# mackelab/poisson-gpfa

Hardware: AMD Instinct MI355X
Metric: EM iterations/sec (higher is better)
Workload: dtype f64

## Files before the change

### poisson-gpfa_amd/csrc/core.hip

```cpp
#include "ctx.h"
#include "model.h"
#include "dual.h"

using namespace pgpfa;

thread_local std::string g_err;
thread_local unsigned long long g_fail_count = 0;

int fail(const char* fmt, ...) {
  char buf[1024];
  va_list ap;
  va_start(ap, fmt);
  vsnprintf(buf, sizeof(buf), fmt, ap);
  va_end(ap);
  g_err = buf;
  ++g_fail_count;
  return 1;
}

int ensure_hbuf(pgpfa_ctx* c, size_t len) {
  if (len <= c->hbuf_len) return 0;
  if (c->hbuf) hipHostFree(c->hbuf);
  c->hbuf = nullptr;
  HIPC(hipHostMalloc((void**)&c->hbuf, len * sizeof(double)));
// ... 827 lines not shown
  {
    const size_t nqmax = (size_t)p * TAU_MULTI_MAX;
    rc |= dmalloc(c, &c->tK, slab * nqmax); rc |= dmalloc(c, &c->tM, slab * nqmax); rc |= dmalloc(c, &c->tA1, slab * nqmax);
    rc |= dmalloc(c, &c->tA2, slab * nqmax);
    rc |= dmalloc(c, &c->tscal, 16 + 8 * nqmax); rc |= dmalloc(c, &c->tpart, 1024 + 64 * nqmax);
  }
  if (rc) { pgpfa_destroy(c); return 1; }
  e = hipStreamSynchronize(c->st);
  if (e != hipSuccess) { pgpfa_destroy(c); return fail("sync: %s", hipGetErrorString(e)); }
  if (const char* g = std::getenv("PGPFA_RANK_GRAN")) { const int v = std::atoi(g); if (v == 4 || v == 8 || v == 16) c->rank_gran = v; }
  c->info["n_pad"] = c->npad;
  c->info["counts_two_bytes"] = 0.0;
  c->info["trial_lengths_set"] = 0.0;
  c->info["observed_set"] = 0.0;
  c->info["observed_bins_set"] = 0.0;
  c->info["last_cd_unobserved_neurons"] = 0.0;
  c->info["arena_bytes"] = 0.0;
  c->info["last_eps_wt_norm"] = 0.0;
  c->info["last_eps_wt_rms"] = 0.0;
  c->info["last_split_cov"] = 0.0;
  c->info["last_syrk_tile"] = 0.0;
  c->info["last_split_sps"] = 0.0;
  c->info["last_cross_kernel"] = 0.0;
  c->info["last_mix_form"] = 0.0;
  c->info["last_yt_mix_fused"] = 0.0;
  c->info["last_cov_f32"] = 0.0;
  c->info["last_cov_f32_fallbacks"] = 0.0;
  for (const char* k : {"plan_ms_total", "plans", "set_params_calls", "last_retry_ms", "last_dense_retries", "last_param_step", "last_param_step_prev",
                        "last_fallback_no_descent", "last_fallback_line_search", "last_fallback_outer_cap", "arena_grow_ms_total", "last_cold_restarts"}) c->info[k] = 0.0;
  *out = c;
  return 0;
}

int pgpfa_destroy(pgpfa_ctx* c) {
  if (!c) return 0;
  hipSetDevice(c->device);
  if (c->st) hipStreamSynchronize(c->st);
  if (c->comm) ncclCommDestroy(c->comm);
  for (void* p : c->allocs) hipFree(p);
  if (c->vsmgp) hipFree(c->vsmgp);
  if (c->Flr32) hipFree(c->Flr32);
  if (c->lam_keep) hipFree(c->lam_keep);
  if (c->split_buf) hipFree(c->split_buf);
  if (c->Yhi) hipFree(c->Yhi);
  if (c->trial_len) hipFree(c->trial_len);
  if (c->obs) hipFree(c->obs);
  if (c->binw) hipFree(c->binw);
  if (c->nlive) hipFree(c->nlive);
  if (c->trunc_q) hipFree(c->trunc_q);
  arena_release(c);
  if (c->hbuf) hipHostFree(c->hbuf);
  if (c->dl_stage) hipHostFree(c->dl_stage);
  if (c->hibuf) hipHostFree(c->hibuf);
  if (c->ring) hipHostFree(c->ring);
  if (c->h_pcg) hipHostFree(c->h_pcg);
  if (c->h_seq) hipHostFree(c->h_seq);
  for (auto e : c->prof.pool) hipEventDestroy(e);
  if (c->st2) { hipStreamSynchronize(c->st2); hipStreamDestroy(c->st2); }
  if (c->tau_pin) hipHostFree(c->tau_pin);
  if (c->ev_tau_fork) hipEventDestroy(c->ev_tau_fork);
  if (c->ev_tau_done) hipEventDestroy(c->ev_tau_done);
  if (c->ev_fork) hipEventDestroy(c->ev_fork);
  if (c->ev_join) hipEventDestroy(c->ev_join);
  if (c->st) hipStreamDestroy(c->st);
  delete c;
  return 0;
}

int pgpfa_set_option(pgpfa_ctx* c, const char* key, double v) {
  if (!c || !key) return fail("null argument");
  const std::string k(key);
  if (k == "newton_xtol") c->xtol = v;
  else if (k == "newton_max_iter") c->max_iter = (int)v;
  else if (k == "use_mfma") {
    const bool was = c->mfma;
    c->mfma = (v != 0.0);
    if (c->have_params && c->rank_gran != 16 && was != c->mfma)
      CHK(pgpfa_set_params(c, std::vector<double>(c->hC).data(), std::vector<double>(c->hd).data(), std::vector<double>(c->htau).data()));
  }
  else if (k == "cd_mfma") c->cd_mfma = (v != 0.0);
  else if (k == "cd_hess_mfma") c->cd_hess_mfma = (v != 0.0);
  else if (k == "cross_kernel") c->cross_kernel = (v != 0.0);
  else if (k == "cd_debug") c->cd_debug = (int)v;
  else if (k == "pcg_fused") c->pcg_fused = (int)v;
  else if (k == "pcg_w32") c->pcg_w32 = (v != 0.0);
  else if (k == "pcg_form") c->pcg_form = (int)v;
  else if (k == "pcg_vec32") c->pcg_vec32 = (int)v;
  else if (k == "pcg_rx32") c->pcg_rx32 = (int)v;
  else if (k == "pcg_adapt") c->pcg_adapt = (int)v;
  else if (k == "pcg_xcd") c->pcg_xcd = (int)v;
  else if (k == "mt_fill") c->mt_fill = (int)v;
  else if (k == "overlap_factors") c->overlap_factors = (int)v;
  else if (k == "mix_slot") c->mix_slot = (int)v;
  else if (k == "yt_mix") c->yt_mix = (v != 0.0);
  else if (k == "pivchol_pairs") c->pivchol_pairs = (v != 0.0);
  else if (k == "vsm_b4") c->vsm_b4 = (int)v;
  else if (k == "poisson_tiles") c->poisson_tiles = (int)v;
  else if (k == "yt_mix_dbg") c->yt_mix_dbg = (int)v;
  else if (k == "yt_mix_dma") c->yt_mix_dma = (v != 0.0);
  else if (k == "syrk_dbg") c->syrk_dbg = (int)v;
  else if (k == "syrk_tile") c->syrk_tile = (int)v;
  else if (k == "mix_wide") c->mix_wide = (int)v;
  else if (k == "thin_products") {
    const bool was = c->thin_products >= 2;
    c->thin_products = (int)v;
// ... 689 lines not shown
```

### poisson-gpfa_amd/csrc/cov.hip

```cpp
#include "ctx.h"
#include "model.h"
#include "split.h"
#include "ytmix.h"

using namespace pgpfa;

template <typename TIN>
void launch_post_vsm(pgpfa_ctx* c, const TIN* Mt, long long sM, int ncol, int ns, int full_range, const int* roff = nullptr, int ts = 0) {
  const int T = c->T, p = c->p;
  if (ts <= 0) ts = T;
  if (p > 10 && c->vsm_mfma) {
    const int CB = post_vsm_mfma_cb(p, sizeof(TIN) == 4);
    if (p <= 20 && c->vsm_b4) {
      constexpr int VW = 16 / (int)sizeof(TIN);
      const bool vec = c->vsm_b4 >= 2 && T % VW == 0 && ts % VW == 0 && c->ld % VW == 0 && sM % VW == 0 && (((size_t)Mt) & 15) == 0;
      auto go = [&](auto nbk, auto vv) {
        constexpr int NBK = decltype(nbk)::value;
        constexpr bool VEC = decltype(vv)::value;
        const size_t lds4 = (size_t)CB * post_vsm_b4_cs(p, VEC) * sizeof(TIN);
        constexpr int BINS = VEC ? 64 : 32;
        (void)hipFuncSetAttribute(reinterpret_cast<const void*>(&post_vsm_b4_kernel<NBK, TIN, VEC>), hipFuncAttributeMaxDynamicSharedMemorySize, (int)lds4);
        hipLaunchKernelGGL((post_vsm_b4_kernel<NBK, TIN, VEC>), dim3((T + BINS - 1) / BINS, ns), dim3(512), lds4, c->st, Mt, sM, c->ld, ncol, T, p, c->vsm,
                           c->ident, c->trial_of_slot, full_range, CB, roff, (int)GBN, ts);
      };
// ... 107 lines not shown
  SyrkF16Args a{};
  a.D = D; a.sD = sD; a.ldd = ldd; a.ts = Ts; a.part = part;
  a.T = T; a.p = p; a.ract = ract; a.nslots = nb; a.sps = sps; a.ngroups = ngroups;
  a.dbg = c->syrk_dbg;
  const int t256 = (T + 255) / 256;
  const bool big = tile_req >= 256 && T > 256 && (Ts & 3) == 0 && (ldd & 3) == 0 && t256 * 256 <= Ts && (((size_t)D) & 15) == 0 && (sD & 3) == 0;
  a.tiles = big ? t256 : (T + 127) / 128; a.ntiles = a.tiles * (a.tiles + 1) / 2;
  const long long blocks = (long long)a.ntiles * ngroups * p;
  prof_begin(c, TAG_VSM, 3.0 * (double)nb * ract * T * T * p);
  if (big) {
    const size_t lds = (size_t)4 * 2 * 256 * 32 * sizeof(_Float16);
    (void)hipFuncSetAttribute(reinterpret_cast<const void*>(&syrk256_f16x2_kernel), hipFuncAttributeMaxDynamicSharedMemorySize, (int)lds);
    hipLaunchKernelGGL(syrk256_f16x2_kernel, dim3((unsigned)blocks), dim3(512), lds, c->st, a);
  } else {
    hipLaunchKernelGGL(syrk_f16x2_kernel, dim3((unsigned)blocks), dim3(256), 0, c->st, a);
  }
  prof_end(c);
  *tile_used = big ? 256 : 128;
  *sps_out = sps;
  *ngroups_out = ngroups;
  return 0;
}

static int split_latent_sums(pgpfa_ctx* c, const double* A0, long long sM, int lda, const float* Dk, long long sD, int ldd, int rk, int kw, int T, int nb, int sps,
                             bool cross, double* Spart, double* Xpart, double* Ssum, double* Xsum, int* cross_used) {
  const int ngroups = (nb + sps - 1) / sps;
  const int spsS = std::max(1, (nb + SPLIT_NS - 1) / SPLIT_NS);
  auto seg = [&](int sper, bool is_x, double* out) -> int {
    const int nfull = nb / sper, rem = nb - nfull * sper;
    for (int part = 0; part < 2; ++part) {
      const int first = part ? nfull * sper : 0, per = part ? rem : sper, ng = part ? (rem ? 1 : 0) : nfull;
      if (ng == 0 || per == 0) continue;
      GemmP g{};
      g.A = A0 + (size_t)first * sM; g.sA = (long long)per * sM; g.lda = lda;
      g.kseg = kw; g.sAseg = sM;
      g.K = per * kw; g.alpha = 1.0; g.beta = 0.0; g.slots = nullptr; g.nbatch = ng; g.kflags = 0; g.bm = 64;
      g.M = rk;
      if (is_x) {
        g.B = reinterpret_cast<const double*>(Dk + (size_t)first * sD);
        g.sB = (long long)per * sD; g.ldb = ldd; g.sBseg = sD; g.b_f32 = 1;
        g.N = T; g.mode = GEMM_FULL;
        g.C = out + (size_t)(part ? nfull : 0) * rk * T; g.sC = (long long)rk * T; g.ldc = rk;
      } else {
        g.B = g.A; g.sB = g.sA; g.ldb = lda; g.sBseg = sM;
        g.N = rk; g.mode = GEMM_LOWER;
        g.C = out + (size_t)(part ? nfull : 0) * rk * rk; g.sC = (long long)rk * rk; g.ldc = rk;
      }
      CHK(gemm(c, false, g));
    }
    return 0;
  };
  CHK(seg(spsS, false, Spart));
  const bool use_cross = cross && c->mfma && rk % 16 == 0 && kw % 16 == 0;
  if (use_cross) {
    for (int row0 = 0; row0 < rk; row0 += 128) {
      CrossArgs ca{};
      ca.A = A0; ca.sM = sM; ca.lda = lda;
      ca.D = Dk; ca.sD = sD; ca.ldd = ldd;
      ca.C = Xpart; ca.sC = (long long)rk * T;
      ca.rk = std::min(128, rk - row0); ca.T = T; ca.kw = kw; ca.nslots = nb; ca.sps = sps;
      ca.row0 = row0; ca.ldc = rk;
      prof_begin(c, TAG_GEMM, 2.0 * (double)nb * ca.rk * (double)kw * T);
      cross_term_launch<float, false>(ca, dim3((T + 63) / 64, ngroups), c->st);
      prof_end(c);
    }
    HIPC(hipGetLastError());
  } else {
    CHK(seg(sps, true, Xpart));
  }
  const int ngS = (nb + spsS - 1) / spsS;
  hipLaunchKernelGGL(sum_groups_kernel, dim3((unsigned)(((size_t)rk * rk + 63) / 64)), dim3(256), 0, c->st, Spart, ngS, rk, rk, 32, Ssum);
  hipLaunchKernelGGL(sum_groups_kernel, dim3((unsigned)(((size_t)rk * T + 63) / 64)), dim3(256), 0, c->st, Xpart, ngroups, rk, T, 0, Xsum);
  *cross_used = use_cross ? 1 : 0;
  return 0;
}

static int accumulate_split(pgpfa_ctx* c, const CholWS& lw, int nb, int ract, int Ts, bool skip_zero_cols, int ctile, bool fused) {
  const int T = c->T, p = c->p, Tp = c->Tp, rpad = c->rpad;
  const long long sW = (long long)T * p * p;
  const size_t tt = (size_t)T * T;
  (void)skip_zero_cols;
  constexpr int NS = SPLIT_NS, NG = PACC_SPLITS + 1;
  const size_t tq = (size_t)round_up(T, 16) * round_up(T, 16);
  if (!c->split_buf) {
    const size_t len = ((size_t)NS + NG + 3) * tq + 2 * (size_t)p * tt + 1024;
    if (hipMalloc((void**)&c->split_buf, len * sizeof(double)) != hipSuccess) { (void)hipGetLastError(); c->split_buf = nullptr; return fail("out of device memory for the split accumulation (%zu bytes)", len * sizeof(double)); }
    c->bytes += len * sizeof(double);
  }
  double* Spart = c->split_buf;
  double* Xpart = Spart + (size_t)NS * tq;
  double* Ssum = Xpart + (size_t)NG * tq;
  double* Xsum = Ssum + tq;
  double* Zb = Xsum + tq;
  double* T1 = Zb + tq;
  double* Xfull = T1 + (size_t)p * tt;
// ... 51 lines not shown
                           c->Gbin, sW, T, ract, c->eps, c->vsm, c->ident, c->trial_of_slot, c->d_roff, ctile, Ts);
        mix_form = 2;
        return;
      }
      if (c->mix_slot) {
        (void)hipFuncSetAttribute(reinterpret_cast<const void*>(&mix_slot_kernel<PW, 256, 2>), hipFuncAttributeMaxDynamicSharedMemorySize, (int)mix_slot_lds(PW, 256));
        hipLaunchKernelGGL((mix_slot_kernel<PW, 256, 2>), dim3((T + 255) / 256, nb), dim3(256), mix_slot_lds(PW, 256), c->st, (const double*)lw.H, (long long)lw.sH, c->ld, D, sD, ldd,
                           c->Gbin, sW, T, p, ract, c->eps, c->vsm, c->ident, c->trial_of_slot, c->d_roff, ctile, Ts);
        mix_form = 1;
        return;
      }
    }
    if constexpr (PW <= 16)
      hipLaunchKernelGGL(mix_vsm_split_kernel<PW>, dim3((T + 63) / 64, nb), dim3(256), 0, c->st, (const double*)lw.H, (long long)lw.sH, c->ld, D, sD, ldd,
                         c->Gbin, sW, T, p, ract, c->eps, c->vsm, c->ident, c->trial_of_slot, c->d_roff, ctile, Ts);
  });
  prof_end(c);
  }
  c->info["last_mix_form"] = (double)mix_form;
  int sps = 0, ngroups = 0, tile_used = 0;
  CHK(split_syrk_launch(c, D, sD, ldd, Ts, T, p, ract, nb, 0, c->syrk_tile, c->ppart, &tile_used, &sps, &ngroups));
  c->info["last_syrk_tile"] = (double)tile_used;
  c->info["last_split_sps"] = (double)sps;
  bool cross_ran = false;
  for (int k = 0; k < p; ++k) {
    const int rk = c->rk[k], r0 = c->roff[k] & ~15;
    const int rrow = c->roff[k];
    const int kw = ract - r0;
    if (kw <= 0 || rk <= 0) {
      HIPC(hipMemsetAsync(T1 + (size_t)k * tt, 0, tt * sizeof(double), c->st));
      HIPC(hipMemsetAsync(Xfull + (size_t)k * tt, 0, tt * sizeof(double), c->st));
      continue;
    }
    const double* A0 = lw.Mt + rrow + (size_t)r0 * rpad;
    int cross_used = 0;
    CHK(split_latent_sums(c, A0, (long long)lw.sM, rpad, D + (size_t)k * Ts + (size_t)r0 * ldd, sD, ldd, rk, kw, T, nb, sps, c->cross_kernel, Spart, Xpart, Ssum, Xsum,
                          &cross_used));
    cross_ran = cross_ran || cross_used != 0;
    const double* Fk = c->Flr + (size_t)k * Tp * Tp;
    GemmP z{};
    z.A = Fk; z.lda = Tp; z.B = Ssum; z.ldb = rk; z.C = Zb; z.ldc = T;
    z.M = T; z.N = rk; z.K = rk; z.alpha = 1.0; z.beta = 0.0; z.nbatch = 1; z.mode = GEMM_FULL;
    CHK(gemm(c, true, z));
    GemmP t1 = z;
    t1.A = Zb; t1.lda = T; t1.B = Fk; t1.ldb = Tp; t1.C = T1 + (size_t)k * tt; t1.ldc = T; t1.N = T;
    CHK(gemm(c, false, t1));
    GemmP xf = z;
    xf.B = Xsum; xf.ldb = rk; xf.C = Xfull + (size_t)k * tt; xf.ldc = T; xf.N = T;
    CHK(gemm(c, true, xf));
  }
  c->info["last_cross_kernel"] = cross_ran ? 1.0 : 0.0;
  {
    const int nt64 = (T + PACC_TS - 1) / PACC_TS;
    hipLaunchKernelGGL(pacc_split_reduce_kernel, dim3(nt64 * (nt64 + 1) / 2, p), dim3(256), 0, c->st, T1, Xfull, c->ppart, ngroups, c->Gbin, sW, nb, c->eps, T, Tp,
                       p, c->Pacc);
  }
  HIPC(hipGetLastError());
  c->pacc_used = true;
  return 0;
}

static int posterior_blocks_lowrank_impl(pgpfa_ctx* c, int nb, bool want_vsmgp, bool accumulate, double* logdet_out, bool allow_lap32, double* ld_dev) {
  const int T = c->T, p = c->p, Tp = c->Tp, pp = p * p;
  const int rpad = c->rpad;
  const int ract = round_up(c->rtot, 16);
  const long long sW = (long long)T * pp;
  c->last_cov_lowrank = true;
  CHK(bin_blocks(c, c->W, sW, c->Gbin, c->Wt, sW, nb, (logdet_out || ld_dev) ? c->ldet_buf : nullptr));
  const bool split_candidate = want_vsmgp && accumulate && c->split_cov && c->mfma && (p <= 16 || (p <= 20 && c->mix_wide));
  unsigned* norm_bits = reinterpret_cast<unsigned*>(c->pcg_ratio);
  if (split_candidate || c->measure_mix) {
    HIPC(hipMemsetAsync(norm_bits, 0, 4 * sizeof(unsigned), c->st));
    const long long nblk = (long long)nb * T;
    hipLaunchKernelGGL(block_norm_max_kernel, dim3((unsigned)std::min<long long>((nblk * p + 255) / 256, 2048)), dim3(256), 0, c->st, c->Wt, nblk, p, c->eps, norm_bits,
// ... 149 lines not shown
    c->info["last_eps_wt_rms"] = std::max(c->info["last_eps_wt_rms"], rms);
    split = split_candidate && std::isfinite(hv) && std::isfinite(rms) && rms <= c->split_max_norm && (double)hv <= 0.9;
    return 0;
  };
  const bool fuse_candidate = split_candidate && c->yt_mix && c->mfma && p <= 10 && (ract == c->rtot || (c->rank_compact && ract <= lw.nact));
  if (fuse_candidate) CHK(decide_split());
  const bool fused = fuse_candidate && split;
  c->info["last_yt_mix_fused"] = fused ? 1.0 : 0.0;
  if (!fused) {
    for (int k = 0; k < p; ++k) {
      const int c0 = skip_zero_cols ? (c->roff[k] / ctile) * ctile : 0;
      if (c0 >= ract) continue;
      GemmP g{};
      g.A = c->Flr + (size_t)k * Tp * Tp; g.sA = 0; g.lda = Tp;
      g.B = lw.Mt + c->roff[k] + (size_t)c0 * rpad; g.sB = lw.sM; g.ldb = rpad;
      g.C = lw.H + (size_t)k * Ts + (size_t)c0 * c->ld; g.sC = lw.sH; g.ldc = c->ld;
      g.M = T; g.N = ract - c0; g.K = c->rk[k]; g.alpha = 1.0; g.beta = 0.0;
      g.slots = c->ident; g.nbatch = nb; g.mode = GEMM_FULL; g.kflags = 0;
      CHK(gemm(c, true, g));
    }
  }
  if (!decided) CHK(decide_split());
  c->info["last_split_cov"] = split ? 1.0 : 0.0;
  if (!split) for (const char* key : {"last_syrk_tile", "last_split_sps", "last_cross_kernel", "last_mix_form"}) c->info[key] = 0.0;
  if (want_vsmgp && split) {
    CHK(accumulate_split(c, lw, nb, ract, Ts, skip_zero_cols, ctile, fused));
  } else if (want_vsmgp) {
    prof_begin(c, TAG_MIX, (double)nb * c->n * ract * 16.0);
    dispatch_pw(p, [&](auto pw) {
      constexpr int PW = decltype(pw)::value;
      if constexpr (PW <= 16) {
        hipLaunchKernelGGL(mix_vsm_kernel<PW>, dim3((T + 63) / 64, nb), dim3(256), 0, c->st, lw.H, lw.sH, c->ld, c->Gbin, sW, T, p, ract, c->eps,
                           c->vsm, c->ident, c->trial_of_slot, c->d_roff, ctile, Ts);
      } else if (c->mix_wide && p <= 20) {
        hipLaunchKernelGGL((mix_vsm_wide2_kernel<20, false>), dim3((T + 63) / 64, nb), dim3(256), 0, c->st, lw.H, (long long)lw.sH, c->ld, c->Gbin, sW, T, p, ract, c->eps,
                           c->vsm, c->ident, c->trial_of_slot, Ts, c->sink, (float*)nullptr, 0LL, 0);
      } else {
        const int bins = wide_bins(p);
        hipLaunchKernelGGL(mix_vsm_wide_kernel, dim3((T + bins - 1) / bins, nb), dim3(bins * 32), wide_lds_bytes(p, bins, 1), c->st, lw.H, lw.sH,
                           c->ld, c->Gbin, sW, T, p, ract, c->eps, c->vsm, c->ident, c->trial_of_slot, bins, Ts);
      }
    });
    prof_end(c);
  } else {
    prof_begin(c, TAG_VSM, (double)nb * c->n * rpad * p);
    launch_post_vsm(c, (const double*)lw.H, (long long)lw.sH, ract, nb, 1, skip_zero_cols ? c->d_roff : nullptr, Ts);
    prof_end(c);
// ... 294 lines not shown
  float* dD = nullptr;
  double* dpart = nullptr;
  CHK(hb.get(&dD, slot * nslots, 1024));
  HIPC(hipMemcpy(dD, D, slot * nslots * sizeof(float), hipMemcpyHostToDevice));
  CHK(hook_output(hb, &dpart, part, np));
  int sps_used = 0;
  CHK(split_syrk_launch(c, dD, (long long)slot, ldd, ts, T, p, ract, nslots, sps, tile, dpart, tile_used, &sps_used, ngroups));
  HIPC(hipGetLastError());
  HIPC(hipStreamSynchronize(c->st));
  return hook_collect("pgpfa_test_split_syrk", dpart, part, np);
}

int pgpfa_test_split_latent_sums(pgpfa_ctx* c, int nslots, int rk, int kw, int T, int lda, long long sM, int row_off, int ldd, long long sD, int sps, int cross_kernel,
                                 const double* A, const float* D, double* Ssum, double* Xsum) {
  if (!c || !A || !D || !Ssum || !Xsum) return fail("null argument");
  if (nslots < 1 || T < 1 || rk < 1 || kw < 1 || sps < 0 || row_off < 0) return fail("invalid sizes");
  if (rk % 16 != 0) return fail("rk = %d is no multiple of 16", rk);
  if (kw % 16 != 0) return fail("kw = %d is no multiple of 16", kw);
  if (lda < row_off + rk) return fail("lda = %d below row_off + rk = %d", lda, row_off + rk);
  if (ldd < T) return fail("ldd = %d below T = %d", ldd, T);
  if (sM < (long long)kw * lda || sD < (long long)kw * ldd) return fail("slot strides below kw columns");
  if (!c->mfma) return fail("the split form runs on the matrix cores (use_mfma = 1)");
  const int sps_eff = sps > 0 ? sps : std::max(1, (nslots + PACC_SPLITS - 1) / PACC_SPLITS);
  const int ng = (nslots + sps_eff - 1) / sps_eff;
  const int spsS = std::max(1, (nslots + SPLIT_NS - 1) / SPLIT_NS), ngS = (nslots + spsS - 1) / spsS;
  HIPC(hipSetDevice(c->device));
  HIPC(hipStreamSynchronize(c->st));
  HookBuffers hb;
  double *dA = nullptr, *dSp = nullptr, *dXp = nullptr, *dS = nullptr, *dX = nullptr;
  float* dD = nullptr;
  CHK(hb.get(&dA, (size_t)sM * nslots, 4096));
  CHK(hb.get(&dD, (size_t)sD * nslots, 4096));
  CHK(hb.get(&dSp, (size_t)ngS * rk * rk, 1024));
  CHK(hb.get(&dXp, (size_t)ng * rk * T, 1024));
  HIPC(hipMemcpy(dA, A, (size_t)sM * nslots * sizeof(double), hipMemcpyHostToDevice));
  HIPC(hipMemcpy(dD, D, (size_t)sD * nslots * sizeof(float), hipMemcpyHostToDevice));
  CHK(hook_output(hb, &dS, Ssum, (size_t)rk * rk));
  CHK(hook_output(hb, &dX, Xsum, (size_t)rk * T));
  int cross_used = 0;
  CHK(split_latent_sums(c, dA + row_off, sM, lda, dD, sD, ldd, rk, kw, T, nslots, sps_eff, cross_kernel != 0, dSp, dXp, dS, dX, &cross_used));
  HIPC(hipGetLastError());
  HIPC(hipStreamSynchronize(c->st));
  if ((cross_kernel != 0) != (cross_used != 0)) return fail("internal: the cross term did not take the requested form");
  CHK(hook_collect("pgpfa_test_split_latent_sums (S)", dS, Ssum, (size_t)rk * rk));
  return hook_collect("pgpfa_test_split_latent_sums (X)", dX, Xsum, (size_t)rk * T);
}
```

### poisson-gpfa_amd/csrc/ctx.h

```cpp
#pragma once
#include <hip/hip_runtime.h>
#include <rccl/rccl.h>

#include <algorithm>
#include <limits>
#include <chrono>
#include <cmath>
#include <cstdarg>
#include <cstdio>
#include <cstring>
#include <deque>
#include <functional>
#include <map>
#include <string>
#include <type_traits>
#include <vector>

#include <mutex>
#include <rocprofiler-sdk-roctx/roctx.h>
#include "../../include/pgpfa.h"
#include "types.h"

using namespace pgpfa;

// ... 186 lines not shown
  bool plan_lowrank = false;
  size_t slab_elems = 0, mt_elems = 0, ws_mark = 0;
  char* arena = nullptr; size_t arena_cap = 0, arena_off = 0; int arena_mode = 0;
  int vmm = 0; size_t va_size = 0, vmm_gran = 0, vmm_granule = (size_t)1 << 30;
  std::vector<std::pair<hipMemGenericAllocationHandle_t, size_t>> vmm_chunks;
  double arena_headroom = 2.0;
  bool mt_dirty = false;
  bool last_cov_lowrank = false;
  bool shared_pcg = true;
  bool pcg_trace = false;
  double* zero16 = nullptr;
  double* sink = nullptr;
  int mix_wide = 1;
  int poisson_tiles = 2;
  int vsm_b4 = 2;
  int pivchol_pairs = 1;
  int yt_mix = 1;
  int syrk_tile = 256;
  int syrk_dbg = 0;
  int yt_mix_dma = 1;
  int yt_mix_dbg = 0;
  int mix_slot = 3;
  bool cross_kernel = true;
  bool measure_mix = false;
  bool time_newton = false;
  int shared_min = 16, pcg_inner_min = 2, pcg_inner_max = 16, pcg_outer_max = 12;
  double pcg_eta0 = 1e-2;
  int splitk_target = 1280;
  int f32_tile64 = 1;
  int small_tile_below = 1 << 30;
  int splitk_below64 = 400;
  double *sc_f = nullptr, *sc_qxx = nullptr, *sc_qdx = nullptr, *sc_qdd = nullptr, *sc_dec = nullptr, *sc_smax = nullptr, *sc_alpha = nullptr;
  int *trial_of_slot = nullptr, *list_a = nullptr, *list_b = nullptr, *ident = nullptr;
  int* mask_of_slot = nullptr;
  bool mask_active = false;
  CholWS kws{};
  double *tK = nullptr, *tM = nullptr, *tA1 = nullptr, *tA2 = nullptr, *tscal = nullptr, *tpart = nullptr;
  double* hbuf = nullptr; size_t hbuf_len = 0;
  struct DlEntry { void* host; size_t off, bytes; };
  PcgCtl fused_ctl_host{};
  char* dl_stage = nullptr; size_t dl_used = 0; std::vector<DlEntry> dl_pending;
  char* dl_stage_dev = nullptr; char* ring_dev = nullptr;
  unsigned* h_seq = nullptr; unsigned* d_seq = nullptr; unsigned seq_next = 0;
  bool copy_kernels = true;
  unsigned long long dl_fail_mark = 0;
  int* hibuf = nullptr; size_t hibuf_len = 0;
// ... 167 lines not shown
```

### poisson-gpfa_amd/csrc/split.h

```cpp
#pragma once
#include <type_traits>
#include <hip/hip_runtime.h>

namespace pgpfa {

typedef _Float16 half8_t __attribute__((ext_vector_type(8)));
typedef float float4v_t __attribute__((ext_vector_type(4)));

constexpr float SPLIT_SCALE = 2048.0f;


template <int PW>
__global__ __launch_bounds__(256, 2) void mix_vsm_split_kernel(const double* __restrict__ Yt, long long sY, int ldy, float* __restrict__ D, long long sD,
                                                            int ldd, const double* __restrict__ G, long long sG, int T, int p, int rpad, double eps,
                                                            double* __restrict__ vsm, const int* __restrict__ slots,
                                                            const int* __restrict__ trial_of_slot, const int* __restrict__ roff, int col_tile, int ts) {
  constexpr int PP = PW * PW, LD = PP + 1, NPAIR = PW * (PW + 1) / 2;
  __shared__ double Gs[64 * LD];
  const int pp = p * p;
  const int slot = slots[blockIdx.y];
  const int t0 = blockIdx.x * 64;
  const int nt = min(64, T - t0);
  const double* gbase = G + (size_t)slot * sG + (size_t)t0 * pp;
  if (p < PW)
// ... 652 lines not shown
  if (!wave_live) return;
  double* C = a.part + (size_t)(k * a.ngroups + g) * a.T * a.T;
  const double inv = 1.0 / ((double)SPLIT_SCALE * (double)SPLIT_SCALE);
#pragma unroll
  for (int mi = 0; mi < 4; ++mi) {
    const int i = i0 + wm * 64 + mi * 16 + l15;
    if (i >= a.T) continue;
#pragma unroll
    for (int ni = 0; ni < 8; ++ni)
#pragma unroll
      for (int r = 0; r < 4; ++r) {
        const int j = j0 + wn * 128 + ni * 16 + 4 * l4 + r;
        if (j >= a.T) continue;
        C[(size_t)j * a.T + i] = (double)acc[mi][ni][r] * inv;
      }
  }
}

struct CrossArgs {
  const double* A; long long sM; int lda;
  const void* D; long long sD; int ldd;
  double* C; long long sC;
  int rk, T, kw, nslots, sps;
  int row0, ldc;
};

template <int NTR, typename TB, bool LOWER>
__global__ __launch_bounds__(256) void cross_term_kernel(CrossArgs a) {
  constexpr int GK = 16;
  constexpr int RS = NTR * 16 + ((NTR & 1) ? 0 : 16);
  constexpr int NA = (GK * NTR * 16 + 255) / 256;
  __shared__ double As[2][GK][RS];
  __shared__ double Bs[2][GK][64 + 16];
  const int tid = threadIdx.x;
  const int lane = tid & 63, wave = __builtin_amdgcn_readfirstlane(tid >> 6);
  const int l15 = lane & 15, l4 = lane >> 4;
  const int t0 = blockIdx.x * 64;
  const int g = blockIdx.y;
  const int s_begin = g * a.sps, s_end = min(a.nslots, s_begin + a.sps);
  const int cps = a.kw / GK;
  const int nchunks = (s_end - s_begin) * cps;
  const int rk = a.rk;
  const TB* Dall = reinterpret_cast<const TB*>(a.D);
  const int ct = blockIdx.x * 4 + wave;
  const bool wave_live = t0 + wave * 16 < a.T;

  double raA[NA], raB[NA];
  TB rbA[4], rbB[4];
  int cur_s = s_begin, cur_c = 0;
  size_t aoff[NA], doff[4];
#pragma unroll
  for (int u = 0; u < NA; ++u) {
    const int e = tid + 256 * u;
    const int kk = min(e / (NTR * 16), GK - 1), i = min(e % (NTR * 16), rk - 1);
    aoff[u] = (size_t)kk * a.lda + i;
  }
#pragma unroll
  for (int u = 0; u < 4; ++u) {
    const int e = tid + 256 * u;
    const int kk = e >> 6, t = min(t0 + (e & 63), a.T - 1) - t0;
    doff[u] = (size_t)kk * a.ldd + t;
  }
  auto load = [&](int, double (&ra)[NA], TB (&rb)[4]) {
    const int c0 = cur_c * GK;
    const double* Ap = a.A + (size_t)cur_s * a.sM + (size_t)c0 * a.lda + a.row0;
    const TB* Dp = Dall + (size_t)cur_s * a.sD + (size_t)c0 * a.ldd + t0;
#pragma unroll
    for (int u = 0; u < NA; ++u) ra[u] = Ap[aoff[u]];
#pragma unroll
    for (int u = 0; u < 4; ++u) rb[u] = Dp[doff[u]];
    if (cur_c + 1 < cps) ++cur_c;
    else if (cur_s + 1 < s_end) { ++cur_s; cur_c = 0; }
  };
  auto store = [&](int buf, const double (&ra)[NA], const TB (&rb)[4]) {
#pragma unroll
    for (int u = 0; u < NA; ++u) {
      const int e = tid + 256 * u;
      const int kk = e / (NTR * 16), i = e - kk * (NTR * 16);
      if (kk < GK) As[buf][kk][i] = (i < rk) ? ra[u] : 0.0;
    }
#pragma unroll
    for (int u = 0; u < 4; ++u) {
      const int e = tid + 256 * u;
      Bs[buf][e >> 6][e & 63] = (t0 + (e & 63) < a.T) ? (double)rb[u] : 0.0;
    }
  };
  mdouble4 acc[NTR];
#pragma unroll
  for (int mi = 0; mi < NTR; ++mi) acc[mi] = mdouble4{0.0, 0.0, 0.0, 0.0};
  auto multiply = [&](int buf) {
    if (!wave_live) return;
#pragma unroll
    for (int kk = 0; kk < GK; kk += 4) {
      const double bf = Bs[buf][kk + l4][wave * 16 + l15];
#pragma unroll
      for (int mi = 0; mi < NTR; ++mi)
        if (!LOWER || mi >= ct) acc[mi] = __builtin_amdgcn_mfma_f64_16x16x4f64(bf, As[buf][kk + l4][mi * 16 + l15], acc[mi], 0, 0, 0);
    }
  };
  if (nchunks > 0) {
    load(0, raA, rbA);
    load(1, raB, rbB);
    store(0, raA, rbA);
  }
  __syncthreads();
  for (int ch = 0; ch < nchunks; ch += 2) {
    load(ch + 2, raA, rbA);
    multiply(0);
    if (ch + 1 < nchunks) store(1, raB, rbB);
    __syncthreads();
    if (ch + 1 >= nchunks) break;
    load(ch + 3, raB, rbB);
    multiply(1);
    if (ch + 2 < nchunks) store(0, raA, rbA);
    __syncthreads();
  }
  if (!wave_live) return;
  double* C = a.C + (size_t)g * a.sC + a.row0;
#pragma unroll
  for (int mi = 0; mi < NTR; ++mi) {
    const int i = mi * 16 + l15;
    if (i >= rk || (LOWER && mi < ct)) continue;
#pragma unroll
    for (int r = 0; r < 4; ++r) {
      const int t = t0 + wave * 16 + l4 + 4 * r;
      if (t < a.T) C[(size_t)t * a.ldc + i] = acc[mi][r];
    }
  }
}

template <typename TB, bool LOWER>
inline void cross_term_launch(const CrossArgs& ca, dim3 grid, hipStream_t st) {
  switch (ca.rk / 16) {
    case 1: hipLaunchKernelGGL((cross_term_kernel<1, TB, LOWER>), grid, dim3(256), 0, st, ca); break;
    case 2: hipLaunchKernelGGL((cross_term_kernel<2, TB, LOWER>), grid, dim3(256), 0, st, ca); break;
    case 3: hipLaunchKernelGGL((cross_term_kernel<3, TB, LOWER>), grid, dim3(256), 0, st, ca); break;
    case 4: hipLaunchKernelGGL((cross_term_kernel<4, TB, LOWER>), grid, dim3(256), 0, st, ca); break;
    case 5: hipLaunchKernelGGL((cross_term_kernel<5, TB, LOWER>), grid, dim3(256), 0, st, ca); break;
    case 6: hipLaunchKernelGGL((cross_term_kernel<6, TB, LOWER>), grid, dim3(256), 0, st, ca); break;
    case 7: hipLaunchKernelGGL((cross_term_kernel<7, TB, LOWER>), grid, dim3(256), 0, st, ca); break;
    default: hipLaunchKernelGGL((cross_term_kernel<8, TB, LOWER>), grid, dim3(256), 0, st, ca); break;
  }
}

inline __global__ __launch_bounds__(256) void sum_groups_kernel(const double* __restrict__ part, int ngroups, int M, int N, int lower, double* __restrict__ out) {
  __shared__ double red[4][64];
  const int el = threadIdx.x & 63, q = threadIdx.x >> 6;
  const size_t e = (size_t)blockIdx.x * 64 + el;
  const bool in = e < (size_t)M * N;
  const size_t ec = in ? e : 0;
  const int i = (int)(ec % M), j = (int)(ec / M);
  const size_t src = (lower > 0 && (i / lower) < (j / lower)) ? (size_t)i * M + j : ec;
  const size_t gs = (size_t)M * N;
  double s8[8] = {0.0, 0.0, 0.0, 0.0, 0.0, 0.0, 0.0, 0.0};
  int g = q;
  for (; g + 28 < ngroups; g += 32) {
    double v[8];
#pragma unroll
    for (int u = 0; u < 8; ++u) v[u] = part[(size_t)(g + 4 * u) * gs + src];
#pragma unroll
    for (int u = 0; u < 8; ++u) s8[u] += v[u];
  }
  for (; g < ngroups; g += 4) s8[0] += part[(size_t)g * gs + src];
  red[q][el] = ((s8[0] + s8[1]) + (s8[2] + s8[3])) + ((s8[4] + s8[5]) + (s8[6] + s8[7]));
  __syncthreads();
  if (q == 0 && in) out[e] = (red[0][el] + red[1][el]) + (red[2][el] + red[3][el]);
}

constexpr int PACC_TS = 32;
inline __global__ __launch_bounds__(256) void pacc_split_reduce_kernel(const double* __restrict__ T1, const double* __restrict__ X, const double* __restrict__ DD, int ngroups,
                                                                const double* __restrict__ G, long long sG, int nslots, double eps, int T, int Tp, int p,
                                                                double* __restrict__ Pacc) {
  constexpr int TS = PACC_TS;
  __shared__ double Xa[TS][TS + 1], Xb[TS][TS + 1], Ss[TS][TS + 1];
  __shared__ double gd[TS];
  const int k = blockIdx.y;
  int tj = 0, rem = blockIdx.x;
  const int ntile = (T + TS - 1) / TS;
  while (rem >= ntile - tj) { rem -= ntile - tj; ++tj; }
  const int ti = tj + rem;
  const int i0 = ti * TS, j0 = tj * TS;
  const size_t tt = (size_t)T * T;
  const double* t1 = T1 + (size_t)k * tt;
  const double* x = X + (size_t)k * tt;
  const double* dd = DD + (size_t)k * ngroups * tt;
  double* out = Pacc + (size_t)k * Tp * Tp;
  const int tid = threadIdx.x;
  for (int e = tid; e < TS * TS; e += 256) {
    const int r = e % TS, cc = e / TS;
// ... 40 lines not shown
```

Baseline: 12.49.

## Size cross-term groups to occupancy, widen column tiles, batch split tail GEMMs

```diff
diff --git a/poisson-gpfa_amd/csrc/core.hip b/poisson-gpfa_amd/csrc/core.hip
--- a/poisson-gpfa_amd/csrc/core.hip
+++ b/poisson-gpfa_amd/csrc/core.hip
@@ -873,6 +873,7 @@
   c->info["last_syrk_tile"] = 0.0;
   c->info["last_split_sps"] = 0.0;
   c->info["last_cross_kernel"] = 0.0;
+  c->info["last_cross_groups"] = 0.0;
   c->info["last_mix_form"] = 0.0;
   c->info["last_yt_mix_fused"] = 0.0;
   c->info["last_cov_f32"] = 0.0;
@@ -893,6 +894,7 @@
   if (c->Flr32) hipFree(c->Flr32);
   if (c->lam_keep) hipFree(c->lam_keep);
   if (c->split_buf) hipFree(c->split_buf);
+  if (c->split_tail) hipFree(c->split_tail);
   if (c->Yhi) hipFree(c->Yhi);
   if (c->trial_len) hipFree(c->trial_len);
   if (c->obs) hipFree(c->obs);
@@ -932,6 +934,10 @@
   else if (k == "cd_mfma") c->cd_mfma = (v != 0.0);
   else if (k == "cd_hess_mfma") c->cd_hess_mfma = (v != 0.0);
   else if (k == "cross_kernel") c->cross_kernel = (v != 0.0);
+  else if (k == "cross_groups") c->cross_groups = std::max(0, (int)v);
+  else if (k == "cross_xcd") c->cross_xcd = (v != 0.0) ? 1 : 0;
+  else if (k == "cross_bins") c->cross_bins = (v >= 128.0) ? 128 : 64;
+  else if (k == "split_tail_batched") c->split_tail_batched = (v != 0.0) ? 1 : 0;
   else if (k == "cd_debug") c->cd_debug = (int)v;
   else if (k == "pcg_fused") c->pcg_fused = (int)v;
   else if (k == "pcg_w32") c->pcg_w32 = (v != 0.0);
diff --git a/poisson-gpfa_amd/csrc/cov.hip b/poisson-gpfa_amd/csrc/cov.hip
--- a/poisson-gpfa_amd/csrc/cov.hip
+++ b/poisson-gpfa_amd/csrc/cov.hip
@@ -153,9 +153,32 @@
   return 0;
 }
 
+static bool split_use_cross(const pgpfa_ctx* c, bool cross, int rk, int kw) { return cross && c->mfma && rk % 16 == 0 && kw % 16 == 0; }
+
+static int split_x_groups(pgpfa_ctx* c, bool use_cross, int rk, int T, int nb, int sps, long long cap, int* spsx) {
+  if (!use_cross) { *spsx = sps; return (nb + sps - 1) / sps; }
+  int want = c->cross_groups;
+  if (want <= 0) {
+    if (c->num_cu <= 0) {
+      int n = 0;
+      if (hipDeviceGetAttribute(&n, hipDeviceAttributeMultiprocessorCount, c->device) != hipSuccess) { (void)hipGetLastError(); n = 0; }
+      c->num_cu = n > 0 ? n : 256;
+    }
+    const int rk0 = std::min(rk, 128), nct = cross_term_nct(rk0, T, c->cross_bins);
+    const int occ = std::max(1, cross_term_occupancy<float, false>(rk0 / 16, nct));
+    const int nbt = (T + 64 * nct - 1) / (64 * nct);
+    want = round_up((c->num_cu * occ + nbt - 1) / nbt, 8);
+  }
+  want = (int)std::max<long long>(1, std::min<long long>(std::min<long long>(want, nb), cap));
+  *spsx = (nb + want - 1) / want;
+  return (nb + *spsx - 1) / *spsx;
+}
+
 static int split_latent_sums(pgpfa_ctx* c, const double* A0, long long sM, int lda, const float* Dk, long long sD, int ldd, int rk, int kw, int T, int nb, int sps,
-                             bool cross, double* Spart, double* Xpart, double* Ssum, double* Xsum, int* cross_used) {
-  const int ngroups = (nb + sps - 1) / sps;
+                             bool cross, long long xcap, double* Spart, double* Xpart, double* Ssum, double* Xsum, int ldo, bool merge_sums, int* cross_used) {
+  const bool use_cross = split_use_cross(c, cross, rk, kw);
+  int spsx = sps;
+  const int ngroups = split_x_groups(c, use_cross, rk, T, nb, sps, xcap, &spsx);
   const int spsS = std::max(1, (nb + SPLIT_NS - 1) / SPLIT_NS);
   auto seg = [&](int sper, bool is_x, double* out) -> int {
     const int nfull = nb / sper, rem = nb - nfull * sper;
@@ -182,26 +205,34 @@
     return 0;
   };
   CHK(seg(spsS, false, Spart));
-  const bool use_cross = cross && c->mfma && rk % 16 == 0 && kw % 16 == 0;
   if (use_cross) {
     for (int row0 = 0; row0 < rk; row0 += 128) {
       CrossArgs ca{};
       ca.A = A0; ca.sM = sM; ca.lda = lda;
       ca.D = Dk; ca.sD = sD; ca.ldd = ldd;
       ca.C = Xpart; ca.sC = (long long)rk * T;
-      ca.rk = std::min(128, rk - row0); ca.T = T; ca.kw = kw; ca.nslots = nb; ca.sps = sps;
+      ca.rk = std::min(128, rk - row0); ca.T = T; ca.kw = kw; ca.nslots = nb; ca.sps = spsx;
+      ca.nct = cross_term_nct(ca.rk, T, c->cross_bins);
+      ca.ngroups = ngroups; ca.nbt = (T + 64 * ca.nct - 1) / (64 * ca.nct); ca.xcd = c->cross_xcd;
       ca.row0 = row0; ca.ldc = rk;
       prof_begin(c, TAG_GEMM, 2.0 * (double)nb * ca.rk * (double)kw * T);
-      cross_term_launch<float, false>(ca, dim3((T + 63) / 64, ngroups), c->st);
+      cross_term_launch<float, false>(ca, c->st);
       prof_end(c);
     }
     HIPC(hipGetLastError());
+    c->info["last_cross_groups"] = (double)ngroups;
   } else {
     CHK(seg(sps, true, Xpart));
   }
   const int ngS = (nb + spsS - 1) / spsS;
-  hipLaunchKernelGGL(sum_groups_kernel, dim3((unsigned)(((size_t)rk * rk + 63) / 64)), dim3(256), 0, c->st, Spart, ngS, rk, rk, 32, Ssum);
-  hipLaunchKernelGGL(sum_groups_kernel, dim3((unsigned)(((size_t)rk * T + 63) / 64)), dim3(256), 0, c->st, Xpart, ngroups, rk, T, 0, Xsum);
+  const SumGroupsJob js{Spart, ngS, rk, rk, 32, Ssum, ldo}, jx{Xpart, ngroups, rk, T, 0, Xsum, ldo};
+  const unsigned nblkS = (unsigned)(((size_t)rk * rk + 63) / 64), nblkX = (unsigned)(((size_t)rk * T + 63) / 64);
+  if (merge_sums) {
+    hipLaunchKernelGGL(sum_groups_kernel, dim3(nblkS + nblkX), dim3(256), 0, c->st, js, jx, (int)nblkS);
+  } else {
+    hipLaunchKernelGGL(sum_groups_kernel, dim3(nblkS), dim3(256), 0, c->st, js, js, (int)nblkS);
+    hipLaunchKernelGGL(sum_groups_kernel, dim3(nblkX), dim3(256), 0, c->st, jx, jx, (int)nblkX);
+  }
   *cross_used = use_cross ? 1 : 0;
   return 0;
 }
@@ -299,21 +330,43 @@
   CHK(split_syrk_launch(c, D, sD, ldd, Ts, T, p, ract, nb, 0, c->syrk_tile, c->ppart, &tile_used, &sps, &ngroups));
   c->info["last_syrk_tile"] = (double)tile_used;
   c->info["last_split_sps"] = (double)sps;
+  int rmax = 0;
+  for (int k = 0; k < p; ++k) rmax = std::max(rmax, c->rk[k]);
+  const bool batched = c->split_tail_batched && rmax > 0 && rmax <= Tp;
+  const size_t sS = (size_t)rmax * rmax, sX = (size_t)rmax * T;
+  if (batched) {
+    const size_t ra = (size_t)std::min(round_up(rmax, 64), std::max(rmax, round_up(T, 16)));
+    const size_t need = (size_t)p * (ra * ra + 2 * ra * T) + 1024;
+    if (need > c->split_tail_len) {
+      if (c->split_tail) { HIPC(hipStreamSynchronize(c->st)); HIPC(hipFree(c->split_tail)); c->bytes -= c->split_tail_len * sizeof(double); c->split_tail = nullptr; c->split_tail_len = 0; }
+      if (hipMalloc((void**)&c->split_tail, need * sizeof(double)) != hipSuccess) { (void)hipGetLastError(); c->split_tail = nullptr; return fail("out of device memory for the batched tail of the split accumulation (%zu bytes)", need * sizeof(double)); }
+      c->split_tail_len = need;
+      c->bytes += need * sizeof(double);
+    }
+    HIPC(hipMemsetAsync(c->split_tail, 0, (size_t)p * (sS + sX) * sizeof(double), c->st));
+  }
+  double* SsumB = c->split_tail;
+  double* XsumB = batched ? SsumB + (size_t)p * sS : nullptr;
+  double* ZB = batched ? XsumB + (size_t)p * sX : nullptr;
+  const long long xcap = (long long)NG * (long long)tq;
   bool cross_ran = false;
   for (int k = 0; k < p; ++k) {
     const int rk = c->rk[k], r0 = c->roff[k] & ~15;
     const int rrow = c->roff[k];
     const int kw = ract - r0;
     if (kw <= 0 || rk <= 0) {
+      if (batched) continue;
       HIPC(hipMemsetAsync(T1 + (size_t)k * tt, 0, tt * sizeof(double), c->st));
       HIPC(hipMemsetAsync(Xfull + (size_t)k * tt, 0, tt * sizeof(double), c->st));
       continue;
     }
     const double* A0 = lw.Mt + rrow + (size_t)r0 * rpad;
     int cross_used = 0;
-    CHK(split_latent_sums(c, A0, (long long)lw.sM, rpad, D + (size_t)k * Ts + (size_t)r0 * ldd, sD, ldd, rk, kw, T, nb, sps, c->cross_kernel, Spart, Xpart, Ssum, Xsum,
-                          &cross_used));
+    CHK(split_latent_sums(c, A0, (long long)lw.sM, rpad, D + (size_t)k * Ts + (size_t)r0 * ldd, sD, ldd, rk, kw, T, nb, sps, c->cross_kernel,
+                          xcap / ((long long)rk * T), Spart, Xpart, batched ? SsumB + (size_t)k * sS : Ssum, batched ? XsumB + (size_t)k * sX : Xsum,
+                          batched ? rmax : rk, batched, &cross_used));
     cross_ran = cross_ran || cross_used != 0;
+    if (batched) continue;
     const double* Fk = c->Flr + (size_t)k * Tp * Tp;
     GemmP z{};
     z.A = Fk; z.lda = Tp; z.B = Ssum; z.ldb = rk; z.C = Zb; z.ldc = T;
@@ -326,7 +379,20 @@
     xf.B = Xsum; xf.ldb = rk; xf.C = Xfull + (size_t)k * tt; xf.ldc = T; xf.N = T;
     CHK(gemm(c, true, xf));
   }
+  if (batched) {
+    GemmP z{};
+    z.A = c->Flr; z.sA = (long long)Tp * Tp; z.lda = Tp; z.B = SsumB; z.sB = (long long)sS; z.ldb = rmax; z.C = ZB; z.sC = (long long)sX; z.ldc = T;
+    z.M = T; z.N = rmax; z.K = rmax; z.alpha = 1.0; z.beta = 0.0; z.slots = nullptr; z.nbatch = p; z.mode = GEMM_FULL;
+    CHK(gemm(c, true, z));
+    GemmP t1 = z;
+    t1.A = ZB; t1.sA = (long long)sX; t1.lda = T; t1.B = c->Flr; t1.sB = (long long)Tp * Tp; t1.ldb = Tp; t1.C = T1; t1.sC = (long long)tt; t1.ldc = T; t1.N = T;
+    CHK(gemm(c, false, t1));
+    GemmP xf = z;
+    xf.B = XsumB; xf.sB = (long long)sX; xf.ldb = rmax; xf.C = Xfull; xf.sC = (long long)tt; xf.ldc = T; xf.N = T;
+    CHK(gemm(c, true, xf));
+  }
   c->info["last_cross_kernel"] = cross_ran ? 1.0 : 0.0;
+  if (!cross_ran) c->info["last_cross_groups"] = 0.0;
   {
     const int nt64 = (T + PACC_TS - 1) / PACC_TS;
     hipLaunchKernelGGL(pacc_split_reduce_kernel, dim3(nt64 * (nt64 + 1) / 2, p), dim3(256), 0, c->st, T1, Xfull, c->ppart, ngroups, c->Gbin, sW, nb, c->eps, T, Tp,
@@ -522,7 +588,7 @@
   }
   if (!decided) CHK(decide_split());
   c->info["last_split_cov"] = split ? 1.0 : 0.0;
-  if (!split) for (const char* key : {"last_syrk_tile", "last_split_sps", "last_cross_kernel", "last_mix_form"}) c->info[key] = 0.0;
+  if (!split) for (const char* key : {"last_syrk_tile", "last_split_sps", "last_cross_kernel", "last_cross_groups", "last_mix_form"}) c->info[key] = 0.0;
   if (want_vsmgp && split) {
     CHK(accumulate_split(c, lw, nb, ract, Ts, skip_zero_cols, ctile, fused));
   } else if (want_vsmgp) {
@@ -863,9 +929,11 @@
   if (sM < (long long)kw * lda || sD < (long long)kw * ldd) return fail("slot strides below kw columns");
   if (!c->mfma) return fail("the split form runs on the matrix cores (use_mfma = 1)");
   const int sps_eff = sps > 0 ? sps : std::max(1, (nslots + PACC_SPLITS - 1) / PACC_SPLITS);
-  const int ng = (nslots + sps_eff - 1) / sps_eff;
   const int spsS = std::max(1, (nslots + SPLIT_NS - 1) / SPLIT_NS), ngS = (nslots + spsS - 1) / spsS;
   HIPC(hipSetDevice(c->device));
+  const long long xcap = std::max(1, nslots);
+  int spsx = 0;
+  const int ng = split_x_groups(c, split_use_cross(c, cross_kernel != 0, rk, kw), rk, T, nslots, sps_eff, xcap, &spsx);
   HIPC(hipStreamSynchronize(c->st));
   HookBuffers hb;
   double *dA = nullptr, *dSp = nullptr, *dXp = nullptr, *dS = nullptr, *dX = nullptr;
@@ -879,7 +947,7 @@
   CHK(hook_output(hb, &dS, Ssum, (size_t)rk * rk));
   CHK(hook_output(hb, &dX, Xsum, (size_t)rk * T));
   int cross_used = 0;
-  CHK(split_latent_sums(c, dA + row_off, sM, lda, dD, sD, ldd, rk, kw, T, nslots, sps_eff, cross_kernel != 0, dSp, dXp, dS, dX, &cross_used));
+  CHK(split_latent_sums(c, dA + row_off, sM, lda, dD, sD, ldd, rk, kw, T, nslots, sps_eff, cross_kernel != 0, xcap, dSp, dXp, dS, dX, rk, false, &cross_used));
   HIPC(hipGetLastError());
   HIPC(hipStreamSynchronize(c->st));
   if ((cross_kernel != 0) != (cross_used != 0)) return fail("internal: the cross term did not take the requested form");
diff --git a/poisson-gpfa_amd/csrc/ctx.h b/poisson-gpfa_amd/csrc/ctx.h
--- a/poisson-gpfa_amd/csrc/ctx.h
+++ b/poisson-gpfa_amd/csrc/ctx.h
@@ -232,6 +232,13 @@
   int yt_mix_dbg = 0;
   int mix_slot = 3;
   bool cross_kernel = true;
+  int cross_groups = 0;
+  int cross_xcd = 1;
+  int cross_bins = 128;
+  int split_tail_batched = 1;
+  int num_cu = 0;
+  double* split_tail = nullptr;
+  size_t split_tail_len = 0;
   bool measure_mix = false;
   bool time_newton = false;
   int shared_min = 16, pcg_inner_min = 2, pcg_inner_max = 16, pcg_outer_max = 12;
diff --git a/poisson-gpfa_amd/csrc/split.h b/poisson-gpfa_amd/csrc/split.h
--- a/poisson-gpfa_amd/csrc/split.h
+++ b/poisson-gpfa_amd/csrc/split.h
@@ -698,33 +698,48 @@
   const void* D; long long sD; int ldd;
   double* C; long long sC;
   int rk, T, kw, nslots, sps;
+  int ngroups, nbt, xcd;
+  int nct;
   int row0, ldc;
 };
 
-template <int NTR, typename TB, bool LOWER>
+template <int NTR, typename TB, bool LOWER, int NCT = 1>
 __global__ __launch_bounds__(256) void cross_term_kernel(CrossArgs a) {
+  static_assert(NCT == 1 || (NCT == 2 && !LOWER), "two column tiles per wave: the cross term only");
   constexpr int GK = 16;
   constexpr int RS = NTR * 16 + ((NTR & 1) ? 0 : 16);
   constexpr int NA = (GK * NTR * 16 + 255) / 256;
+  constexpr int BW = 64 * NCT;
+  constexpr int NBV = GK * BW / 256;
+  typedef typename std::conditional<NCT == 2, TB, double>::type TS;
   __shared__ double As[2][GK][RS];
-  __shared__ double Bs[2][GK][64 + 16];
+  __shared__ TS Bs[2][GK][BW + 16];
   const int tid = threadIdx.x;
   const int lane = tid & 63, wave = __builtin_amdgcn_readfirstlane(tid >> 6);
   const int l15 = lane & 15, l4 = lane >> 4;
-  const int t0 = blockIdx.x * 64;
-  const int g = blockIdx.y;
+  int bt, g;
+  {
+    const int id = blockIdx.x;
+    if (a.xcd) { const int m = id >> 3; const int q = m / a.nbt; bt = m - q * a.nbt; g = (id & 7) + 8 * q; }
+    else { g = id / a.nbt; bt = id - g * a.nbt; }
+  }
+  if (g >= a.ngroups) return;
+  const int t0 = bt * BW;
   const int s_begin = g * a.sps, s_end = min(a.nslots, s_begin + a.sps);
   const int cps = a.kw / GK;
   const int nchunks = (s_end - s_begin) * cps;
   const int rk = a.rk;
   const TB* Dall = reinterpret_cast<const TB*>(a.D);
-  const int ct = blockIdx.x * 4 + wave;
-  const bool wave_live = t0 + wave * 16 < a.T;
+  const int ct = bt * 4 + wave;
+  bool live[NCT];
+#pragma unroll
+  for (int c = 0; c < NCT; ++c) live[c] = t0 + c * 64 + wave * 16 < a.T;
+  const bool wave_live = live[0];
 
   double raA[NA], raB[NA];
-  TB rbA[4], rbB[4];
+  TB rbA[NBV], rbB[NBV];
   int cur_s = s_begin, cur_c = 0;
-  size_t aoff[NA], doff[4];
+  size_t aoff[NA], doff[NBV];
 #pragma unroll
   for (int u = 0; u < NA; ++u) {
     const int e = tid + 256 * u;
@@ -732,23 +747,23 @@
     aoff[u] = (size_t)kk * a.lda + i;
   }
 #pragma unroll
-  for (int u = 0; u < 4; ++u) {
+  for (int u = 0; u < NBV; ++u) {
     const int e = tid + 256 * u;
-    const int kk = e >> 6, t = min(t0 + (e & 63), a.T - 1) - t0;
+    const int kk = e / BW, t = min(t0 + (e % BW), a.T - 1) - t0;
     doff[u] = (size_t)kk * a.ldd + t;
   }
-  auto load = [&](int, double (&ra)[NA], TB (&rb)[4]) {
+  auto load = [&](int, double (&ra)[NA], TB (&rb)[NBV]) {
     const int c0 = cur_c * GK;
     const double* Ap = a.A + (size_t)cur_s * a.sM + (size_t)c0 * a.lda + a.row0;
     const TB* Dp = Dall + (size_t)cur_s * a.sD + (size_t)c0 * a.ldd + t0;
 #pragma unroll
     for (int u = 0; u < NA; ++u) ra[u] = Ap[aoff[u]];
 #pragma unroll
-    for (int u = 0; u < 4; ++u) rb[u] = Dp[doff[u]];
+    for (int u = 0; u < NBV; ++u) rb[u] = Dp[doff[u]];
     if (cur_c + 1 < cps) ++cur_c;
     else if (cur_s + 1 < s_end) { ++cur_s; cur_c = 0; }
   };
-  auto store = [&](int buf, const double (&ra)[NA], const TB (&rb)[4]) {
+  auto store = [&](int buf, const double (&ra)[NA], const TB (&rb)[NBV]) {
 #pragma unroll
     for (int u = 0; u < NA; ++u) {
       const int e = tid + 256 * u;
@@ -756,22 +771,31 @@
       if (kk < GK) As[buf][kk][i] = (i < rk) ? ra[u] : 0.0;
     }
 #pragma unroll
-    for (int u = 0; u < 4; ++u) {
+    for (int u = 0; u < NBV; ++u) {
       const int e = tid + 256 * u;
-      Bs[buf][e >> 6][e & 63] = (t0 + (e & 63) < a.T) ? (double)rb[u] : 0.0;
-    }
-  };
-  mdouble4 acc[NTR];
-#pragma unroll
-  for (int mi = 0; mi < NTR; ++mi) acc[mi] = mdouble4{0.0, 0.0, 0.0, 0.0};
+      Bs[buf][e / BW][e % BW] = (t0 + (e % BW) < a.T) ? (TS)rb[u] : (TS)0;
+    }
+  };
+  mdouble4 acc[NCT][NTR];
+#pragma unroll
+  for (int c = 0; c < NCT; ++c)
+#pragma unroll
+    for (int mi = 0; mi < NTR; ++mi) acc[c][mi] = mdouble4{0.0, 0.0, 0.0, 0.0};
   auto multiply = [&](int buf) {
     if (!wave_live) return;
 #pragma unroll
     for (int kk = 0; kk < GK; kk += 4) {
-      const double bf = Bs[buf][kk + l4][wave * 16 + l15];
-#pragma unroll
-      for (int mi = 0; mi < NTR; ++mi)
-        if (!LOWER || mi >= ct) acc[mi] = __builtin_amdgcn_mfma_f64_16x16x4f64(bf, As[buf][kk + l4][mi * 16 + l15], acc[mi], 0, 0, 0);
+      double bf[NCT];
+#pragma unroll
+      for (int c = 0; c < NCT; ++c) bf[c] = (double)Bs[buf][kk + l4][c * 64 + wave * 16 + l15];
+#pragma unroll
+      for (int mi = 0; mi < NTR; ++mi) {
+        if (LOWER && mi < ct) continue;
+        const double af = As[buf][kk + l4][mi * 16 + l15];
+#pragma unroll
+        for (int c = 0; c < NCT; ++c)
+          if (c == 0 || live[c]) acc[c][mi] = __builtin_amdgcn_mfma_f64_16x16x4f64(bf[c], af, acc[c][mi], 0, 0, 0);
+      }
     }
   };
   if (nchunks > 0) {
@@ -794,35 +818,78 @@
   if (!wave_live) return;
   double* C = a.C + (size_t)g * a.sC + a.row0;
 #pragma unroll
-  for (int mi = 0; mi < NTR; ++mi) {
-    const int i = mi * 16 + l15;
-    if (i >= rk || (LOWER && mi < ct)) continue;
-#pragma unroll
-    for (int r = 0; r < 4; ++r) {
-      const int t = t0 + wave * 16 + l4 + 4 * r;
-      if (t < a.T) C[(size_t)t * a.ldc + i] = acc[mi][r];
-    }
-  }
-}
+  for (int c = 0; c < NCT; ++c)
+#pragma unroll
+    for (int mi = 0; mi < NTR; ++mi) {
+      const int i = mi * 16 + l15;
+      if (i >= rk || (LOWER && mi < ct)) continue;
+#pragma unroll
+      for (int r = 0; r < 4; ++r) {
+        const int t = t0 + c * 64 + wave * 16 + l4 + 4 * r;
+        if (t < a.T) C[(size_t)t * a.ldc + i] = acc[c][mi][r];
+      }
+    }
+}
+
+inline unsigned cross_term_grid(const CrossArgs& ca) { return (unsigned)((ca.xcd ? (ca.ngroups + 7) / 8 * 8 : ca.ngroups) * ca.nbt); }
+
+template <typename TB, bool LOWER, typename F>
+inline void cross_term_dispatch(int ntr, int nct, F&& f) {
+  if constexpr (!LOWER && std::is_same<TB, float>::value) {
+    if (nct == 2) {
+      switch (ntr) {
+        case 1: f(&cross_term_kernel<1, TB, LOWER, 2>); return;
+        case 2: f(&cross_term_kernel<2, TB, LOWER, 2>); return;
+        case 3: f(&cross_term_kernel<3, TB, LOWER, 2>); return;
+        case 4: f(&cross_term_kernel<4, TB, LOWER, 2>); return;
+        default: break;
+      }
+    }
+  }
+  switch (ntr) {
+    case 1: f(&cross_term_kernel<1, TB, LOWER>); break;
+    case 2: f(&cross_term_kernel<2, TB, LOWER>); break;
+    case 3: f(&cross_term_kernel<3, TB, LOWER>); break;
+    case 4: f(&cross_term_kernel<4, TB, LOWER>); break;
+    case 5: f(&cross_term_kernel<5, TB, LOWER>); break;
+    case 6: f(&cross_term_kernel<6, TB, LOWER>); break;
+    case 7: f(&cross_term_kernel<7, TB, LOWER>); break;
+    default: f(&cross_term_kernel<8, TB, LOWER>); break;
+  }
+}
+
+inline int cross_term_nct(int rk, int T, int bins_req) { return (bins_req >= 128 && rk <= 64 && T > 64) ? 2 : 1; }
 
 template <typename TB, bool LOWER>
-inline void cross_term_launch(const CrossArgs& ca, dim3 grid, hipStream_t st) {
-  switch (ca.rk / 16) {
-    case 1: hipLaunchKernelGGL((cross_term_kernel<1, TB, LOWER>), grid, dim3(256), 0, st, ca); break;
-    case 2: hipLaunchKernelGGL((cross_term_kernel<2, TB, LOWER>), grid, dim3(256), 0, st, ca); break;
-    case 3: hipLaunchKernelGGL((cross_term_kernel<3, TB, LOWER>), grid, dim3(256), 0, st, ca); break;
-    case 4: hipLaunchKernelGGL((cross_term_kernel<4, TB, LOWER>), grid, dim3(256), 0, st, ca); break;
-    case 5: hipLaunchKernelGGL((cross_term_kernel<5, TB, LOWER>), grid, dim3(256), 0, st, ca); break;
-    case 6: hipLaunchKernelGGL((cross_term_kernel<6, TB, LOWER>), grid, dim3(256), 0, st, ca); break;
-    case 7: hipLaunchKernelGGL((cross_term_kernel<7, TB, LOWER>), grid, dim3(256), 0, st, ca); break;
-    default: hipLaunchKernelGGL((cross_term_kernel<8, TB, LOWER>), grid, dim3(256), 0, st, ca); break;
-  }
-}
-
-inline __global__ __launch_bounds__(256) void sum_groups_kernel(const double* __restrict__ part, int ngroups, int M, int N, int lower, double* __restrict__ out) {
+inline void cross_term_launch(const CrossArgs& ca, hipStream_t st) {
+  const dim3 grid(cross_term_grid(ca));
+  cross_term_dispatch<TB, LOWER>(ca.rk / 16, ca.nct, [&](auto kern) { hipLaunchKernelGGL(kern, grid, dim3(256), 0, st, ca); });
+}
+
+template <typename TB, bool LOWER>
+inline int cross_term_occupancy(int ntr, int nct) {
+  static int cache[3][9] = {};
+  ntr = ntr < 1 ? 1 : (ntr > 8 ? 8 : ntr);
+  nct = (nct == 2 && ntr <= 4) ? 2 : 1;
+  if (cache[nct][ntr] > 0) return cache[nct][ntr];
+  int n = 0;
+  hipError_t e = hipSuccess;
+  cross_term_dispatch<TB, LOWER>(ntr, nct, [&](auto kern) { e = hipOccupancyMaxActiveBlocksPerMultiprocessor(&n, kern, 256, 0); });
+  if (e != hipSuccess) { (void)hipGetLastError(); return 0; }
+  cache[nct][ntr] = n;
+  return n;
+}
+
+struct SumGroupsJob { const double* part; int ngroups, M, N, lower; double* out; int ldo; };
+inline __global__ __launch_bounds__(256) void sum_groups_kernel(SumGroupsJob j0, SumGroupsJob j1, int nblk0) {
   __shared__ double red[4][64];
+  const bool second = (int)blockIdx.x >= nblk0;
+  const SumGroupsJob& jb = second ? j1 : j0;
+  const double* __restrict__ part = jb.part;
+  double* __restrict__ out = jb.out;
+  const int ngroups = jb.ngroups, M = jb.M, N = jb.N, lower = jb.lower;
   const int el = threadIdx.x & 63, q = threadIdx.x >> 6;
-  const size_t e = (size_t)blockIdx.x * 64 + el;
+  const size_t e = (size_t)(second ? blockIdx.x - nblk0 : blockIdx.x) * 64 + el;
   const bool in = e < (size_t)M * N;
   const size_t ec = in ? e : 0;
   const int i = (int)(ec % M), j = (int)(ec / M);
@@ -840,7 +907,7 @@
   for (; g < ngroups; g += 4) s8[0] += part[(size_t)g * gs + src];
   red[q][el] = ((s8[0] + s8[1]) + (s8[2] + s8[3])) + ((s8[4] + s8[5]) + (s8[6] + s8[7]));
   __syncthreads();
-  if (q == 0 && in) out[e] = (red[0][el] + red[1][el]) + (red[2][el] + red[3][el]);
+  if (q == 0 && in) out[(size_t)j * jb.ldo + i] = (red[0][el] + red[1][el]) + (red[2][el] + red[3][el]);
 }
 
 constexpr int PACC_TS = 32;
```

Measured after the change: 12.51, median of 6. Within noise of the previous version (+0.2%).
